# kjenike/panagram

Hardware: AMD Instinct MI355X
Metric: anchored k-mers/sec building pan-kmer bitmap (higher is better)
Workload: dtype u64

## Files before the change

### panagram_amd/csrc/pg_anchor.hip

```cpp
#include "pg_kernels.h"

#ifndef PG_ANCHOR_PART
#define PG_ANCHOR_PART -1
#endif
#define PG_HAS_PART(n) (PG_ANCHOR_PART == -1 || PG_ANCHOR_PART == (n))
#define PG_MAIN_PART (PG_ANCHOR_PART <= 0)
#if defined(PG_PHASE_TIMING) && PG_ANCHOR_PART != -1
#error "a -DPG_PHASE_TIMING build keeps its counters in one device variable: compile pg_anchor.hip as ONE unit (PG_ANCHOR_PART unset)"
#endif

namespace pg {

hipError_t probe_part0(hipStream_t s, uint32_t w, uint32_t ntiles, const SubTable &st, const uint64_t *seqw, const uint32_t *nmw, const uint32_t *has_n,
                       const SeqDesc *sd, const AnchorDesc *ad, const uint32_t *tile_contig, const uint32_t *sched, uint32_t tile_base, uint8_t *out1,
                       uint32_t nbytes, const RowCols &rc, int rowmode, const FuseArgs *fuse);
hipError_t probe_part1(hipStream_t s, uint32_t w, uint32_t ntiles, const SubTable &st, const uint64_t *seqw, const uint32_t *nmw, const uint32_t *has_n,
                       const SeqDesc *sd, const AnchorDesc *ad, const uint32_t *tile_contig, const uint32_t *sched, uint32_t tile_base, uint8_t *out1,
                       uint32_t nbytes, const RowCols &rc, int rowmode, const FuseArgs *fuse);
hipError_t probe_part2(hipStream_t s, uint32_t w, uint32_t ntiles, const SubTable &st, const uint64_t *seqw, const uint32_t *nmw, const uint32_t *has_n,
                       const SeqDesc *sd, const AnchorDesc *ad, const uint32_t *tile_contig, const uint32_t *sched, uint32_t tile_base, uint8_t *out1,
                       uint32_t nbytes, const RowCols &rc, int rowmode, const FuseArgs *fuse);
hipError_t insert_part0(hipStream_t s, uint32_t win, uint32_t ntiles, const SubTable &st, int w, uint32_t bits, uint32_t count_mode, const uint64_t *seqw,
                        const uint32_t *nmw, const uint32_t *has_n, const SeqDesc *sd, const uint32_t *tile0, uint32_t ncontigs,
                        unsigned long long *counters, uint32_t max_probe);
// ... 363 lines not shown
        for (uint32_t bb = 0; bb < rc.nb1; ++bb) row[rc.col0 + 4 + bb] = (uint8_t)(m1 >> (8 * bb));
    }
}

__device__ __forceinline__ uint32_t lane_up1(uint32_t v) {
    return (uint32_t)__builtin_amdgcn_update_dpp((int)v, (int)v, 0x138 , 0xf, 0xf, false);
}
__device__ __forceinline__ unsigned long long differs_from_lane_below(uint32_t v) {
    uint32_t t;
    asm("s_nop 1\n\tv_xor_b32_dpp %0, %1, %1 wave_shr:1 row_mask:0xf bank_mask:0xf" : "=&v"(t) : "v"(v));
    return __builtin_amdgcn_ballot_w64(t != 0u);
}
#define PG_DPPMIN "s_nop 1\n\tv_min_u32_dpp %0, %0, %1 wave_shr:1 row_mask:0xf bank_mask:0xf\n\t"
template <int W>
__device__ __forceinline__ uint32_t sliding_min(uint32_t x) {
    uint32_t m = x;
    if constexpr (W == 2) asm(PG_DPPMIN : "+v"(m) : "v"(x));
    if constexpr (W == 3) asm(PG_DPPMIN PG_DPPMIN : "+v"(m) : "v"(x));
    if constexpr (W == 4) asm(PG_DPPMIN PG_DPPMIN PG_DPPMIN : "+v"(m) : "v"(x));
    if constexpr (W == 5) asm(PG_DPPMIN PG_DPPMIN PG_DPPMIN PG_DPPMIN : "+v"(m) : "v"(x));
    if constexpr (W == 6) asm(PG_DPPMIN PG_DPPMIN PG_DPPMIN PG_DPPMIN PG_DPPMIN : "+v"(m) : "v"(x));
    if constexpr (W == 7) asm(PG_DPPMIN PG_DPPMIN PG_DPPMIN PG_DPPMIN PG_DPPMIN PG_DPPMIN : "+v"(m) : "v"(x));
    if constexpr (W == 8) asm(PG_DPPMIN PG_DPPMIN PG_DPPMIN PG_DPPMIN PG_DPPMIN PG_DPPMIN PG_DPPMIN : "+v"(m) : "v"(x));
    static_assert(W >= 1 && W <= 8, "minimizer window");
    return m;
}
#undef PG_DPPMIN
__device__ __forceinline__ uint32_t suffix_min8_row(uint32_t x) {
    uint32_t r = x;
    asm("s_nop 1\n\tv_min_u32_dpp %0, %0, %0 row_shl:1 row_mask:0xf bank_mask:0xf\n\t"
        "s_nop 1\n\tv_min_u32_dpp %0, %0, %0 row_shl:2 row_mask:0xf bank_mask:0xf\n\t"
        "s_nop 1\n\tv_min_u32_dpp %0, %0, %0 row_shl:4 row_mask:0xf bank_mask:0xf"
        : "+v"(r));
    return r;
}
#define PG_F "v_min_u32_dpp %0, %0, %0 wave_shr:1 row_mask:0xf bank_mask:0xf\n\t"
#define PG_S(n) "v_min_u32_dpp %1, %1, %1 row_shl:" #n " row_mask:0xf bank_mask:0xf\n\t"
#define PG_N0 "s_nop 0\n\t"
#define PG_N1 "s_nop 1\n\t"
template <int W>
__device__ __forceinline__ uint32_t sliding_min_suffix(uint32_t x, uint32_t &suffix) {
    uint32_t m = x, r = suffix;
    static_assert(W >= 2 && W <= 8, "minimizer window");
    if constexpr (W == 2) asm(PG_N1 PG_F PG_S(1) PG_N1 PG_S(2) PG_N1 PG_S(4) : "+v"(m), "+v"(r));
    if constexpr (W == 3) asm(PG_N1 PG_F PG_S(1) PG_N0 PG_F PG_S(2) PG_N1 PG_S(4) : "+v"(m), "+v"(r));
    if constexpr (W == 4) asm(PG_N1 PG_F PG_S(1) PG_N0 PG_F PG_S(2) PG_N0 PG_F PG_S(4) : "+v"(m), "+v"(r));
    if constexpr (W == 5) asm(PG_N1 PG_F PG_S(1) PG_N0 PG_F PG_S(2) PG_N0 PG_F PG_S(4) PG_N0 PG_F : "+v"(m), "+v"(r));
    if constexpr (W == 6) asm(PG_N1 PG_F PG_S(1) PG_N0 PG_F PG_S(2) PG_N0 PG_F PG_S(4) PG_N0 PG_F PG_N1 PG_F : "+v"(m), "+v"(r));
    if constexpr (W == 7) asm(PG_N1 PG_F PG_S(1) PG_N0 PG_F PG_S(2) PG_N0 PG_F PG_S(4) PG_N0 PG_F PG_N1 PG_F PG_N1 PG_F : "+v"(m), "+v"(r));
    if constexpr (W == 8) asm(PG_N1 PG_F PG_S(1) PG_N0 PG_F PG_S(2) PG_N0 PG_F PG_S(4) PG_N0 PG_F PG_N1 PG_F PG_N1 PG_F PG_N1 PG_F : "+v"(m), "+v"(r));
    suffix = r;
    return m;
}
#undef PG_F
#undef PG_S
#undef PG_N0
#undef PG_N1
__device__ __forceinline__ uint32_t lanes_le_index(unsigned long long mask, uint32_t base) {
    const unsigned long long m1 = mask >> 1;
    const uint32_t c = base + (uint32_t)(mask & 1ull) - 1u;
    return __builtin_amdgcn_mbcnt_hi((uint32_t)(m1 >> 32), __builtin_amdgcn_mbcnt_lo((uint32_t)m1, c));
}

__device__ __forceinline__ uint32_t run_ids(unsigned long long lmask) {
    const uint32_t below = __builtin_amdgcn_mbcnt_hi((uint32_t)(lmask >> 32), __builtin_amdgcn_mbcnt_lo((uint32_t)lmask, ~0u));
    uint32_t rid;
    unsigned long long carry_out;
    asm("v_addc_co_u32_e64 %0, %1, %2, 0, %3" : "=v"(rid), "=s"(carry_out) : "v"(below), "s"(lmask));
    return rid;
}
__device__ __forceinline__ uint32_t set_lane_index(unsigned long long mask, uint32_t base) {
    return __builtin_amdgcn_mbcnt_hi((uint32_t)(mask >> 32), __builtin_amdgcn_mbcnt_lo((uint32_t)mask, base));
}

__device__ __forceinline__ void cols_or_position(unsigned long long *cols, uint32_t pl, uint32_t m0) {
    while (m0) {
        const uint32_t j = (uint32_t)__ffs((int)m0) - 1u;
        m0 &= m0 - 1u;
        atomicOr(&cols[(pl >> 6) * COLS_G + j], 1ull << (pl & 63u));
    }
}

template <bool TWO, int ROWMODE, int SLOTS, int MAXRUN, bool WIDE, int LEVELS, bool INL = false>
__device__ __forceinline__ void drain_queue(const SubTable &st, uint32_t qn, const uint64_t *sw, const uint64_t *rw, uint32_t *q_line,
                                            uint32_t *q_step, uint16_t *q_pl, uint32_t *lines_w, uint4 *buf,
                                            uint8_t *tile_rows, uint32_t nbytes, const RowCols rc, int lane) {
    const int k = (int)st.k;
    constexpr int LDS_LINE_U4 = SLOTS + 1;
    constexpr int STAGE_ITERS = (MAXRUN * SLOTS + 63) / 64;
    const uint8_t *chunk_base = st.buckets + (uint32_t)(lane % SLOTS) * 16u;
    const uint32_t lbytes = INL ? st.layout * 64u : st.slots * (WIDE ? 8u : 16u);
    static_assert(LEVELS >= 1, "k_probe's entries (home line, group) are turned into (next line, step) by level 1's staged batches");
    for (int level = 1; qn > 0; ++level) {
        __syncthreads();
        if (level > LEVELS) {
            for (uint32_t e = lane; e < qn; e += 64) {
                uint32_t m0, m1;
                const uint64_t key = canonical_from_le(extract_bases(sw, q_pl[e]), k);
                if constexpr (WIDE && INL) {
                    uint32_t rw4[4];
                    lane_chase_inl(st, key, (uint32_t)level, q_line[e], q_step[e], rw4);
                    if (rw4[0] | rw4[1] | rw4[2] | rw4[3]) store_row_regs(tile_rows + (uint64_t)q_pl[e] * nbytes, nbytes, rw4);
                } else if constexpr (WIDE) {
                    lane_chase_wide(st, key, (uint32_t)level, q_line[e], q_step[e], m0, m1);
                    if (m1) store_row_wide(st.masks, st.W, nbytes, tile_rows + (uint64_t)q_pl[e] * nbytes, m0, m1);
                } else {
                    lane_chase<TWO, SLOTS>(st, key, (uint32_t)level, q_line[e], q_step[e], m0, m1);
                    if constexpr (ROWMODE == 3) cols_or_position(reinterpret_cast<unsigned long long *>(tile_rows), q_pl[e], m0);
                    else if (m0 | m1) store_row<ROWMODE>(tile_rows + (uint64_t)q_pl[e] * nbytes, m0, m1, rc);
                }
            }
            break;
        }
        uint32_t kept = 0;
        for (uint32_t i0 = 0; i0 < qn; i0 += 64) {
            const uint32_t e = i0 + lane;
            const bool act = e < qn;
            const uint32_t ec = act ? e : qn - 1;
            uint32_t line = q_line[ec], step = q_step[ec];
            if (GROUP_CHAIN > 1 && level == 1) {
                step = step_of_group(step, st.nbuckets);
                line = next_line(line, step, st.nbuckets);
            }
            const uint32_t pl = q_pl[ec];
            const uint64_t kmask = kmer_mask(k);
            const uint64_t X = extract_bases32(reinterpret_cast<const uint32_t *>(sw), pl) & kmask;
            const uint64_t key = canonical_from_xb(X, revcomp_window(rw, pl, kmask, PROBE_SEQ_BASES - (uint32_t)k), k);
            const uint32_t prev_line = lane_up1(line);
            const bool leader = act && (lane == 0 || line != prev_line);
            const unsigned long long lmask = __builtin_amdgcn_ballot_w64(leader);
            const uint32_t rid = lanes_le_index(lmask, 0u);
            const uint32_t nruns = (uint32_t)__popcll(lmask);
            uint32_t m0 = 0, m1 = 0;
            [[maybe_unused]] uint32_t rw4[4] = {0, 0, 0, 0};
            int rcode = 0;
            const uint32_t padline = lmask ? (uint32_t)__builtin_amdgcn_readlane((int)line, __builtin_ctzll(lmask)) : 0u;
            for (uint32_t r0 = 0; r0 < nruns; r0 += MAXRUN) {
                const uint32_t nl = min((uint32_t)MAXRUN, nruns - r0);
                if (lane < MAXRUN) lines_w[lane] = padline;
                if (leader && rid - r0 < nl) lines_w[rid - r0] = line;
                __syncthreads();
                uint4 v[STAGE_ITERS];
                uint32_t ln[STAGE_ITERS];
#pragma unroll
                for (int u = 0; u < STAGE_ITERS; ++u) ln[u] = lines_w[u * (64 / SLOTS) + lane / SLOTS];
#pragma unroll
                for (int u = 0; u < STAGE_ITERS; ++u) v[u] = *reinterpret_cast<const uint4 *>(chunk_base + (uint64_t)ln[u] * lbytes);
#pragma unroll
                for (int u = 0; u < STAGE_ITERS; ++u) {
                    const uint32_t idx = u * 64 + lane;
                    if constexpr (WIDE) buf[(idx / SLOTS) * LDS_LINE_U4 + (idx % SLOTS)] = v[u];
                    else stage_chunk(buf + (idx / SLOTS) * LDS_LINE_U4, idx % SLOTS, SLOTS, v[u]);
                }
                __syncthreads();
                if (act && rid - r0 < nl) {
                    if constexpr (WIDE && INL) {
                        rcode = scan_keys_inl(buf + (rid - r0) * LDS_LINE_U4, key, st.slots, m1);
                        if (m1) masks_inl(buf + (rid - r0) * LDS_LINE_U4, st.slots, st.W, m1 - 1u, rw4);
                    } else if constexpr (WIDE) {
                        rcode = scan_keys16_lds(buf + (rid - r0) * LDS_LINE_U4, key, m1);
                        m0 = line;
                    } else {
                        rcode = scan_line_lds<TWO, SLOTS>(buf + (rid - r0) * LDS_LINE_U4, key, m0, m1);
                    }
                }
                __syncthreads();
            }
            const bool again = act && rcode < 0;
            if constexpr (WIDE && INL) {
                if (act && m1) store_row_regs(tile_rows + (uint64_t)pl * nbytes, nbytes, rw4);
            } else if constexpr (WIDE) {
                if (act && m1) store_row_wide(st.masks, st.W, nbytes, tile_rows + (uint64_t)pl * nbytes, m0, m1);
            } else {
                if constexpr (ROWMODE == 3) {
                    if (act) cols_or_position(reinterpret_cast<unsigned long long *>(tile_rows), pl, m0);
                } else {
                    if (act && (m0 | m1)) store_row<ROWMODE>(tile_rows + (uint64_t)pl * nbytes, m0, m1, rc);
                }
            }
            const unsigned long long kmask2 = __builtin_amdgcn_ballot_w64(again);
            if (again) {
                const uint32_t slot = set_lane_index(kmask2, kept);
                uint32_t nl2 = line, ns2 = step;
                if constexpr (LEVELS + 1 < (int)GROUP_CHAIN) nl2 = next_line(line, step, st.nbuckets);
                else advance_line(key, (uint32_t)level + 1, st.nbuckets, nl2, ns2);
                q_line[slot] = nl2;
                q_step[slot] = ns2;
                q_pl[slot] = (uint16_t)pl;
            }
            kept += (uint32_t)__popcll(kmask2);
            __syncthreads();
        }
        qn = kept;
    }
}

#ifndef PG_FUSE_LOAD_SC1
#define PG_FUSE_LOAD_SC1 1
#endif
typedef const __attribute__((address_space(1))) uint8_t *GlobalBytes;
template <int NW>
__device__ __forceinline__ void fuse_load_row(GlobalBytes base, uint32_t off, uint32_t (&w)[NW]) {
    GlobalBytes p = base + off;
#if PG_FUSE_LOAD_SC1
#pragma unroll
    for (int i = 0; i + 1 < NW; i += 2) {
        const unsigned long long v = __hip_atomic_load(reinterpret_cast<const __attribute__((address_space(1))) unsigned long long *>(p + 4 * i), __ATOMIC_RELAXED,
                                                       __HIP_MEMORY_SCOPE_AGENT);
        w[i] = (uint32_t)v, w[i + 1] = (uint32_t)(v >> 32);
    }
    if constexpr (NW & 1)
        w[NW - 1] = __hip_atomic_load(reinterpret_cast<const __attribute__((address_space(1))) uint32_t *>(p + 4 * (NW - 1)), __ATOMIC_RELAXED, __HIP_MEMORY_SCOPE_AGENT);
#else
    const WordsN<NW> v = *reinterpret_cast<const __attribute__((address_space(1))) WordsN<NW> *>(p);
#pragma unroll
    for (int i = 0; i < NW; ++i) w[i] = v.w[i];
#endif
}
__device__ __forceinline__ void fuse_flush_word(const uint32_t (&pl)[5], uint32_t *out16, int lane) {
    uint32_t R[16];
#pragma unroll
    for (int q = 0; q < 8; ++q) {
        uint32_t v = 0;
#pragma unroll
        for (int i = 0; i < 5; ++i) v |= ((pl[i] >> q) & 0x01010101u) << i;
        R[2 * q] = v & 0x00FF00FFu;
        R[2 * q + 1] = (v >> 8) & 0x00FF00FFu;
    }
#define PG_XCHG(HALF, BIT)                                                  \
    {                                                                       \
        const bool up = (lane & BIT) != 0;                                  \
        _Pragma("unroll") for (int i = 0; i < HALF; ++i) {                  \
            const uint32_t send = up ? R[i] : R[i + HALF];                  \
            const uint32_t keep = up ? R[i + HALF] : R[i];                  \
            R[i] = keep + (uint32_t)__shfl_xor((int)send, BIT);             \
        }                                                                   \
    }
    PG_XCHG(8, 32)
    PG_XCHG(4, 16)
    PG_XCHG(2, 8)
    PG_XCHG(1, 4)
#undef PG_XCHG
    R[0] += (uint32_t)__shfl_xor((int)R[0], 2);
    R[0] += (uint32_t)__shfl_xor((int)R[0], 1);
    if ((lane & 3) == 0) {
        const uint32_t idx = (uint32_t)lane >> 2;
        out16[(idx >> 1) + ((idx & 1u) ? 8u : 0u)] = R[0];
    }
}
template <int NWP, bool LASTPASS>
__device__ __forceinline__ void tile_statistics_pass(uint32_t *Hc, GlobalBytes rs, uint32_t npos, uint32_t nbytes, uint32_t woff,
                                                     uint32_t keep_last, uint32_t split, uint32_t N, uint32_t (&pcs)[4], uint32_t *cs_out, int lane) {
    const uint32_t N1 = N + 1u;
    uint32_t ones[NWP], twos[NWP], fours[NWP], eights[NWP], sixteens[NWP], hold4[NWP], hold8[NWP];
#pragma unroll
    for (int w = 0; w < NWP; ++w) ones[w] = twos[w] = fours[w] = eights[w] = sixteens[w] = hold4[w] = hold8[w] = 0;
    uint32_t nx[4][NWP];
    auto request = [&](int g, uint32_t (&dst)[4][NWP]) __attribute__((always_inline)) {
#pragma unroll
        for (int i = 0; i < 4; ++i) {
            const uint32_t r = (uint32_t)(4 * g + i) * 64u + (uint32_t)lane;
            fuse_load_row<NWP>(rs, min(r, npos - 1u) * nbytes + woff, dst[i]);
        }
    };
    request(0, nx);
#pragma unroll
    for (int g = 0; g < 4; ++g) {
        uint32_t rw[4][NWP];
#pragma unroll
        for (int i = 0; i < 4; ++i)
// ... 53 lines not shown
        const uint32_t pl[5] = {ones[w], twos[w], fours[w], eights[w], sixteens[w]};
        fuse_flush_word(pl, cs_out + 16 * w, lane);
    }
}

template <int NW>
__device__ __forceinline__ void tile_statistics(uint32_t *H, const uint8_t *tile_rows, uint32_t npos, uint32_t nbytes, const AnchorDesc &a,
                                                uint32_t tile_start, uint32_t tile, const FuseArgs &fo, int lane) {
    const uint32_t N = fo.ngenomes, N1 = N + 1u, hw = fo.hw;
    const uint32_t nh = 2u * N1;
#ifdef PG_PHASE_TIMING
    uint32_t tph[5] = {0, 0, 0, 0, 0}, tph_t = (uint32_t)__builtin_readcyclecounter();
#define PG_TPH(i) { const uint32_t n_ = (uint32_t)__builtin_readcyclecounter(); tph[i] += n_ - tph_t; tph_t = n_; }
#else
#define PG_TPH(i)
#endif
    __builtin_amdgcn_s_waitcnt(0x0F70);
    __syncthreads();
    PG_TPH(0)
    const uint64_t base = reinterpret_cast<uint64_t>(tile_rows);
    GlobalBytes rs = reinterpret_cast<GlobalBytes>(((uint64_t)(uint32_t)__builtin_amdgcn_readfirstlane((int)(uint32_t)(base >> 32)) << 32) |
                                                   (uint32_t)__builtin_amdgcn_readfirstlane((int)(uint32_t)base));
    const uint32_t r100 = (100u - tile_start % 100u) % 100u + 100u * (uint32_t)lane;
    const bool want100 = fo.out100 != nullptr && r100 < npos;
    uint32_t w100[NW];
    fuse_load_row<NW>(rs, min(r100, npos - 1u) * nbytes, w100);
    for (uint32_t i = lane; i < 4u * nh; i += 64) H[i] = 0;
    const uint64_t bin_end = ((uint64_t)(tile_start / a.binlen) + 1u) * a.binlen;
    const uint32_t split = (uint32_t)min((uint64_t)npos, bin_end - tile_start);
    const uint32_t keep = (nbytes & 3u) ? ((1u << (8u * (nbytes & 3u))) - 1u) : ~0u;
    uint32_t *const Hc = H + ((uint32_t)lane & 3u) * nh;
    uint32_t *cs_out = fo.tile_cs + (uint64_t)tile * fo.csw;
    uint32_t pcs[4] = {0, 0, 0, 0};
    __syncthreads();
    PG_TPH(1)
    if constexpr (NW <= 2) {
        tile_statistics_pass<NW, true>(Hc, rs, npos, nbytes, 0u, keep, split, N, pcs, cs_out, lane);
        PG_TPH(2)
    } else {
        tile_statistics_pass<2, false>(Hc, rs, npos, nbytes, 0u, ~0u, split, N, pcs, cs_out, lane);
        PG_TPH(2)
        tile_statistics_pass<NW - 2, true>(Hc, rs, npos, nbytes, 8u, keep, split, N, pcs, cs_out + 32, lane);
    }
    if (want100) {
        uint8_t *dst = fo.out100 + a.out100_off + (uint64_t)((tile_start + r100) / 100u) * nbytes;
#pragma unroll
        for (int i = 0; i < NW; ++i)
#pragma unroll
            for (int b = 0; b < 4; ++b)
                if ((uint32_t)(4 * i + b) < nbytes) dst[4 * i + b] = (uint8_t)(w100[i] >> (8 * b));
    }
    __syncthreads();
    PG_TPH(3)
    uint32_t *th = fo.tile_hist + (uint64_t)tile * hw;
    for (uint32_t i = lane; i < hw; i += 64) {
        const uint32_t lo = H[2u * i] + H[nh + 2u * i] + H[2u * nh + 2u * i] + H[3u * nh + 2u * i];
        const uint32_t hi = H[2u * i + 1u] + H[nh + 2u * i + 1u] + H[2u * nh + 2u * i + 1u] + H[3u * nh + 2u * i + 1u];
        th[i] = lo | (hi << 16);
    }
    PG_TPH(4)
#ifdef PG_PHASE_TIMING
    if (lane == 0)
        for (int i = 0; i < 5; ++i) atomicAdd(&pg_phase_cycles[(blockIdx.x & 1023u) * 16u + 11 + i], (unsigned long long)tph[i]);
#endif
#undef PG_TPH
}

template <bool TWO, int ROWMODE, int SLOTS, bool WIDE>
constexpr bool probe_pipelined = SLOTS == 8 && !WIDE && ROWMODE != 3 && (ROWMODE == 1 || ROWMODE >= 4 || TWO);
template <int W_C, bool TWO, int ROWMODE, int SLOTS, bool M64, bool WIDE = false, bool INL = false, bool FUSE = false>
__global__ __launch_bounds__(64, ((probe_pipelined<TWO, ROWMODE, SLOTS, WIDE> || INL || FUSE) ? 8 : 1))
__attribute__((amdgpu_num_sgpr(80))) void k_probe(const SubTable st, const uint64_t *__restrict__ seqw,
                                              const uint32_t *__restrict__ nmw, const uint32_t *__restrict__ has_n,
                                              const SeqDesc *__restrict__ sd, const AnchorDesc *__restrict__ ad,
                                              const uint32_t *__restrict__ tile_contig,
                                              const uint32_t *__restrict__ sched, uint32_t tile_base,
                                              uint8_t *__restrict__ out1, uint32_t nbytes, const RowCols rc, const FuseArgs fo) {
    constexpr int LDS_LINE_U4 = SLOTS + 1;
    constexpr int MAXRUN = PROBE_MAXRUN;
    constexpr int STAGE_ITERS = (MAXRUN * SLOTS + 63) / 64;
    constexpr int BUF_U4 = ((STAGE_ITERS * 64 + SLOTS - 1) / SLOTS) * LDS_LINE_U4;
    constexpr int OFF_RW = PROBE_SEQW * 8, OFF_NW = OFF_RW + (PROBE_SEQW + 1) * 8, OFF_LW = OFF_NW + PROBE_SEQW * 4;
    constexpr int QCAP = PROBE_QCAP;
    constexpr int OFF_BUF = (OFF_LW + MAXRUN * 4 + 15) & ~15, OFF_QL = OFF_BUF + BUF_U4 * 16, OFF_QS = OFF_QL + QCAP * 4;
    constexpr int OFF_QP = OFF_QS + QCAP * 4, LDS_BYTES = OFF_QP + QCAP * 2;
    static_assert(OFF_LW <= 1020 || PROBE_TILE > 1024, "the sequence words must stay within reach of ds_read2_b32's offsets");
    __shared__ __attribute__((aligned(16))) uint8_t lds[LDS_BYTES];
    uint64_t *const sw = reinterpret_cast<uint64_t *>(lds);
    uint64_t *const rw = reinterpret_cast<uint64_t *>(lds + OFF_RW);
    uint32_t *const nw = reinterpret_cast<uint32_t *>(lds + OFF_NW);
    uint32_t(*const lines_w)[MAXRUN] = reinterpret_cast<uint32_t(*)[MAXRUN]>(lds + OFF_LW);
    uint4(*const buf)[BUF_U4] = reinterpret_cast<uint4(*)[BUF_U4]>(lds + OFF_BUF);
    uint32_t *const q_line = reinterpret_cast<uint32_t *>(lds + OFF_QL);
    uint32_t *const q_step = reinterpret_cast<uint32_t *>(lds + OFF_QS);
    uint16_t *const q_pl = reinterpret_cast<uint16_t *>(lds + OFF_QP);
    PG_PH_DECL
    const int lane = threadIdx.x;
    const int k = (int)st.k;
    if constexpr (W_C != 0) __builtin_assume(k >= 20 && k <= 32);
    const uint32_t tile = sched ? sched[blockIdx.x + tile_base] : blockIdx.x + tile_base;
    const uint32_t c = tile_contig[tile];
    const AnchorDesc a = ad[c];
    const SeqDesc s = sd[c];
    const uint32_t tile_start = (tile - a.tile0) * PROBE_TILE;
    const uint32_t npos = min((uint32_t)PROBE_TILE, a.nkmers - tile_start);
    const bool hasn = has_n[c] != 0;

    for (int i = lane; i < PROBE_SEQW; i += 64) {
        const uint64_t wi = (uint64_t)(tile_start >> 5) + i;
        const uint64_t wv = wi < s.nwords ? seqw[s.seq_off + wi] : 0ull;
        sw[i] = wv;
        rw[PROBE_SEQW - 1 - i] = pair_reverse64(~wv);
        nw[i] = (hasn && wi < s.nwords) ? nmw[s.seq_off + wi] : 0u;
    }
    if (lane == 0) rw[PROBE_SEQW] = 0;
    __syncthreads();

    const uint64_t kmask = W_C ? (((uint64_t)(k == 32 ? ~0u : ((1u << (2 * k - 32)) - 1u)) << 32) | 0xFFFFFFFFull) : kmer_mask(k);
    const uint32_t rcb = PROBE_SEQ_BASES - (uint32_t)k;
    constexpr int HALO = W_C ? W_C - 1 : 0;
    constexpr bool CARRY = W_C >= 2;
    constexpr bool CUT = W_C != 0;
    const uint32_t m = W_C ? (uint32_t)k - W_C + 1 : 0;
    const uint64_t mm64 = (m >= 32) ? ~0ull : ((1ull << (2 * (m ? m : 1))) - 1);
    __shared__ unsigned long long cols[ROWMODE == 3 ? TILE_SLOTS * COLS_G : 1];
    if constexpr (ROWMODE == 3) {
        for (uint32_t i = lane; i < TILE_SLOTS * COLS_G; i += 64) cols[i] = 0;
        __syncthreads();
    }
#if PG_ABLATE == 9 || PG_ABLATE == 10
    uint8_t *tile_rows = out1 + (uint64_t)(blockIdx.x & 255u) * PROBE_TILE * nbytes;
#else
    uint8_t *tile_rows = ROWMODE == 3 ? reinterpret_cast<uint8_t *>(cols) : out1 + a.out_off + (uint64_t)tile_start * nbytes;
#endif
    uint32_t qn = 0;

    const uint8_t *chunk_base = st.buckets + (uint32_t)(lane % SLOTS) * 16u;
    const uint32_t lbytes = INL ? st.layout * 64u : st.slots * (WIDE ? 8u : 16u);

    struct Front {
        uint64_t key;
        uint32_t grp, line, rid, nruns, padline;
        uint32_t adv;
        uint32_t ln[STAGE_ITERS];
        unsigned long long rmask, amask, lmask;
    };
    auto carry_at = [&](const uint32_t b0) __attribute__((always_inline)) {
        uint32_t y = ~0u;
        if constexpr (CARRY) {
            const uint32_t q = b0 + (uint32_t)min(lane, HALO - 1);
            const uint64_t fa = extract_bases32(reinterpret_cast<const uint32_t *>(sw), q) & mm64;
            const uint64_t fr = extract_bases32(reinterpret_cast<const uint32_t *>(rw), PROBE_SEQ_BASES - q - m) & mm64;
            const uint32_t h = M64 ? mmer_rank(fa < fr ? fa : fr) : mz_order(min((uint32_t)fa, (uint32_t)fr));
            y = h;
        }
        return y;
    };
    uint32_t carry = ~0u;
    auto front = [&](const uint32_t b0) __attribute__((always_inline)) {
        Front f;
        const int32_t pl = (int32_t)(b0 + lane);
        f.rmask = __builtin_amdgcn_ballot_w64(pl < (int32_t)npos);
        const uint32_t pq = (uint32_t)pl;
        const uint64_t X = extract_bases32(reinterpret_cast<const uint32_t *>(sw), pq) & kmask;
        const uint64_t B = revcomp_window(rw, pq, kmask, rcb);
        f.key = ~(X > B ? X : B) & kmask;
        f.amask = f.rmask;
        if (hasn) f.amask &= __builtin_amdgcn_ballot_w64(extract_nmask(nw, pq, k) == 0);
        [[maybe_unused]] uint32_t own = 0;
        if (W_C) {
            constexpr uint32_t off = (uint32_t)HALO;
            if constexpr (!M64) {
                const uint32_t mm32 = (uint32_t)mm64;
                const uint32_t fa = __builtin_amdgcn_alignbit((uint32_t)(X >> 32), (uint32_t)X, 2 * off) & mm32;
                const uint32_t fr = __builtin_amdgcn_alignbit((uint32_t)(B >> 32), (uint32_t)B, 2 * (HALO - off)) & mm32;
                f.grp = mz_order(min(fa, fr));
            } else {
// ... 51 lines not shown
        return f;
    };
    struct Lines {
        uint4 v[STAGE_ITERS];
    };
    auto issue = [&](const Front &f, const uint32_t r0) __attribute__((always_inline)) {
        Lines L;
        uint32_t ln[STAGE_ITERS];
        if (r0 != 0u) {
            const uint32_t nl = min((uint32_t)MAXRUN, f.nruns - r0);
            const bool leader = __builtin_amdgcn_inverse_ballot_w64(f.lmask);
            if (lane < MAXRUN) lines_w[0][lane] = f.padline;
            if (leader && f.rid - r0 < nl) lines_w[0][f.rid - r0] = f.line;
            __syncthreads();
        }
#pragma unroll
        for (int it = 0; it < STAGE_ITERS; ++it) {
            if (r0 != 0u) ln[it] = lines_w[0][it * (64 / SLOTS) + lane / SLOTS];
            else ln[it] = f.ln[it];
#if PG_ABLATE == 1
            ln[it] &= 511u;
#endif
        }
#pragma unroll
        for (int it = 0; it < STAGE_ITERS; ++it) L.v[it] = *reinterpret_cast<const uint4 *>(chunk_base + (uint64_t)ln[it] * lbytes);
        return L;
    };
    auto back = [&](const Front &f, const Lines &L, const uint32_t b0, auto &&after_staging) __attribute__((always_inline)) {
        const bool act = __builtin_amdgcn_inverse_ballot_w64(f.amask), inrange = __builtin_amdgcn_inverse_ballot_w64(f.rmask);
        const int32_t pl = (int32_t)(b0 + lane);
        uint32_t m0 = 0, m1 = 0;
        [[maybe_unused]] uint32_t rw4[4] = {0, 0, 0, 0};
        int rcode = 0;
        auto stage = [&](const Lines &S) __attribute__((always_inline)) {
            uint4 *const mine = buf[0] + ((uint32_t)lane / SLOTS) * LDS_LINE_U4;
#pragma unroll
            for (int it = 0; it < STAGE_ITERS; ++it) {
                if constexpr (WIDE) mine[it * (64 / SLOTS) * LDS_LINE_U4 + ((uint32_t)lane % SLOTS)] = S.v[it];
                else stage_chunk(mine + it * (64 / SLOTS) * LDS_LINE_U4, (uint32_t)lane % SLOTS, SLOTS, S.v[it]);
            }
            __syncthreads();
        };
        auto scan = [&](const uint32_t r0) __attribute__((always_inline)) {
            const uint32_t nl = min((uint32_t)MAXRUN, f.nruns - r0);
#if PG_ABLATE == 5
            if (act && f.rid - r0 < nl) {
                rcode = 1;
                m0 = m1 = reinterpret_cast<const uint32_t *>(buf[0] + (f.rid - r0) * LDS_LINE_U4)[2];
            }
#else
            if (act && f.rid - r0 < nl) {
                if constexpr (WIDE && INL) {
                    rcode = scan_keys_inl(buf[0] + (f.rid - r0) * LDS_LINE_U4, f.key, st.slots, m1);
                    if (m1) masks_inl(buf[0] + (f.rid - r0) * LDS_LINE_U4, st.slots, st.W, m1 - 1u, rw4);
                } else if constexpr (WIDE) {
                    rcode = scan_keys16_lds(buf[0] + (f.rid - r0) * LDS_LINE_U4, f.key, m1);
                    m0 = f.line;
                } else {
                    rcode = scan_line_lds<TWO, SLOTS>(buf[0] + (f.rid - r0) * LDS_LINE_U4, f.key, m0, m1);
                }
            }
#endif
            __syncthreads();
        };
        PG_PH(1)
        __builtin_amdgcn_s_waitcnt(0x0F70);
        PG_PH(2)
        stage(L);
        PG_PH(3)
        after_staging();
        PG_PH(4)
        scan(0u);
        PG_PH(5)
        if constexpr (!CUT)
        for (uint32_t r0 = MAXRUN; r0 < f.nruns; r0 += MAXRUN) {
            const Lines X = issue(f, r0);
            __builtin_amdgcn_s_waitcnt(0x0F70);
            stage(X);
            scan(r0);
        }
        const unsigned long long omask = f.amask & __builtin_amdgcn_sicmp(rcode, 0, 40);
        const bool ovf = __builtin_amdgcn_inverse_ballot_w64(omask);
        if (omask) {
            uint32_t step, nx;
            if constexpr (GROUP_CHAIN == 1) {
                key_sequence(f.key, st.nbuckets, nx, step);
            } else {
                step = f.grp;
                nx = f.line;
            }
            const uint32_t slot = set_lane_index(omask, qn);
            if (ovf) {
                q_line[slot] = nx;
                q_step[slot] = step;
                q_pl[slot] = (uint16_t)pl;
            }
            qn += (uint32_t)__popcll(omask);
        }
        PG_PH(10)
        if constexpr (WIDE && INL) {
            const bool fuse = (nbytes & 3u) != 0u && b0 + (uint32_t)__popcll(f.rmask) < npos;
            if (fuse) {
                const uint32_t mine = inrange ? rw4[0] : 0u;
                const uint32_t nxt = (uint32_t)__builtin_amdgcn_update_dpp(0, (int)mine, 0x130 , 0xf, 0xf, true);
                if (inrange) store_row_fused(tile_rows + (uint64_t)(uint32_t)pl * nbytes, nbytes, rw4, nxt);
            } else if (inrange) {
                store_row_regs(tile_rows + (uint64_t)(uint32_t)pl * nbytes, nbytes, rw4);
            }
        } else if constexpr (WIDE) {
#if PG_ABLATE == 2
            if (inrange && m0 == 0xDEADBEEFu && m1 == 77u)
#elif PG_ABLATE == 8 || PG_ABLATE == 10
            if (m1) m0 = 0, m1 = 1;
            if (inrange)
#else
            if (st.W == 4u && (nbytes & 3u) != 0u && b0 + (uint32_t)__popcll(f.rmask) < npos) {
                uint32_t v4[4] = {0, 0, 0, 0};
                if (inrange && m1) {
                    const WordsN<4> g = *reinterpret_cast<const WordsN<4> *>(reinterpret_cast<const uint32_t *>(st.masks) + ((uint64_t)m0 * SPLIT_KEYS + (m1 - 1u)) * 4u);
                    v4[0] = g.w[0], v4[1] = g.w[1], v4[2] = g.w[2], v4[3] = g.w[3];
                }
                const uint32_t nxt = (uint32_t)__builtin_amdgcn_update_dpp(0, (int)v4[0], 0x130 , 0xf, 0xf, true);
                if (inrange) store_row_fused(tile_rows + (uint64_t)(uint32_t)pl * nbytes, nbytes, v4, nxt);
            } else if (inrange)
#endif
                store_row_wide(st.masks, st.W, nbytes, tile_rows + (uint64_t)(uint32_t)pl * nbytes, m0, m1);
        } else if constexpr (ROWMODE == 3) {
            const uint32_t w0 = b0 >> 6, sh = b0 & 63u;
            for (uint32_t j = 0; j < rc.col0; ++j) {
                const unsigned long long shifted = __ballot(inrange && ((m0 >> j) & 1u));
                if (lane == 0 && shifted) {
                    cols[w0 * COLS_G + j] |= shifted << sh;
                    if (sh && (shifted >> (64u - sh))) cols[(w0 + 1) * COLS_G + j] |= shifted >> (64u - sh);
                }
            }
        } else {
            if (ROWMODE == 6 && b0 + (uint32_t)__popcll(f.rmask) < npos) {
                const uint32_t mine = inrange ? m0 : 0u;
                const uint32_t nxt = (uint32_t)__builtin_amdgcn_update_dpp(0, (int)mine, 0x130 , 0xf, 0xf, true);
                struct __attribute__((packed)) U32 { uint32_t v; };
                if (inrange) reinterpret_cast<U32 *>(tile_rows + (uint32_t)pl * 3u)->v = (m0 & 0xFFFFFFu) | (nxt << 24);
            } else if constexpr (ROWMODE == 6) {
                const uint32_t nxt = (uint32_t)__builtin_amdgcn_update_dpp(0, (int)m0, 0x130 , 0xf, 0xf, false);
                const uint32_t o4 = (uint32_t)reinterpret_cast<uintptr_t>(tile_rows) & 3u;
                const uint32_t j = ((uint32_t)pl - o4) & 3u;
                const uint32_t lo = (nxt << 24) | (m0 & 0xFFFFFFu);
                const uint32_t dw = __builtin_amdgcn_alignbit(nxt >> 8, lo, 8u * j);
                const unsigned long long nextin = f.rmask >> 1;
                const unsigned long long dmask = f.rmask & nextin & __builtin_amdgcn_ballot_w64(j != 3u);
                const unsigned long long fmask = f.rmask & (1ull | ~nextin);
                uint8_t *row = tile_rows + (uint32_t)pl * 3u;
                if (__builtin_amdgcn_inverse_ballot_w64(dmask)) *reinterpret_cast<uint32_t *>(row + j) = dw;
                if (__builtin_amdgcn_inverse_ballot_w64(fmask)) store_row<ROWMODE>(row, m0, m1, rc);
            } else
#if PG_ABLATE == 2
            if (inrange && m0 == 0xDEADBEEFu)
#else
            if (ROWMODE == 0 && TWO && rc.words == 3u && nbytes >= 5u && b0 + (uint32_t)__popcll(f.rmask) < npos) {
                const uint32_t mine = inrange ? m0 : 0u;
                const uint32_t nxt = (uint32_t)__builtin_amdgcn_update_dpp(0, (int)mine, 0x130 , 0xf, 0xf, true);
                if (inrange) {
                    typedef uint32_t u32x2u __attribute__((ext_vector_type(2), aligned(1)));
                    const uint32_t t8 = 8u * (nbytes - 4u);
                    u32x2u q = {m0, (m1 & ((1u << t8) - 1u)) | (nxt << t8)};
                    *reinterpret_cast<u32x2u *>(tile_rows + (uint32_t)pl * nbytes) = q;
                }
            } else if (inrange)
#endif
                store_row<ROWMODE>(tile_rows + (ROWMODE == 1 ? (uint32_t)pl : ROWMODE == 4 ? (uint32_t)pl * 4u : ROWMODE == 5 ? (uint32_t)pl * 2u : ROWMODE == 6 ? (uint32_t)pl * 3u : (uint32_t)pl * nbytes), m0, m1, rc);
        }
        PG_PH(6)
    };
    constexpr bool PIPE = probe_pipelined<TWO, ROWMODE, SLOTS, WIDE>;
    constexpr int LEVELS = (W_C >= 6 && !TWO && !WIDE && PROBE_STAGED_LEVELS > 1) ? 1 : PROBE_STAGED_LEVELS;
    static_assert(QCAP >= 128, "an early drain must leave room for a batch");
    constexpr uint32_t QROOM = QCAP - 64;
    uint32_t b0 = 0;
    if constexpr (PIPE) {
        Lines L;
#pragma unroll
        for (int it = 0; it < STAGE_ITERS; ++it) L.v[it] = make_uint4(0, 0, 0, 0);
        PG_PH(0)
        carry = carry_at(0u);
        Front cur = front(0u);
        L = issue(cur, 0u);
        for (;;) {
            PG_PH(7)
            const uint32_t b1 = b0 + cur.adv;
            const bool more = b1 < npos;
            Front nxt = cur;
            __builtin_amdgcn_sched_barrier(0);
            if (more) nxt = front(b1);
            __builtin_amdgcn_sched_barrier(0);
            back(cur, L, b0, [&]() __attribute__((always_inline)) {
                if (more) L = issue(nxt, 0u);
            });
            __builtin_amdgcn_sched_barrier(0);
            b0 = b1;
            if (!more || qn > QROOM) break;
            cur = nxt;
        }
    } else {
        {
            carry = carry_at(0u);
            const Front f = front(0u);
            const Lines L = issue(f, 0u);
            back(f, L, 0u, [] {});
            b0 = f.adv;
        }
        while (b0 < npos && qn <= QROOM) {
            const Front f = front(b0);
            const Lines L = issue(f, 0u);
            back(f, L, b0, [] {});
            b0 += f.adv;
        }
    }
    PG_PH(7)
    for (;;) {
        drain_queue<TWO, ROWMODE, SLOTS, MAXRUN, WIDE, LEVELS, INL>(st, qn, sw, rw, q_line, q_step, q_pl, lines_w[0], buf[0], tile_rows, nbytes, rc, lane);
        qn = 0;
        if (b0 >= npos) break;
        __syncthreads();
        carry = carry_at(b0);
        while (b0 < npos && qn <= QROOM) {
            const Front f = front(b0);
            const Lines L = issue(f, 0u);
            back(f, L, b0, [] {});
            b0 += f.adv;
        }
    }
    PG_PH(8)
    PG_PH_FLUSH
    if constexpr (FUSE) {
        static_assert(ROWMODE != 1 && ROWMODE != 3 && LDS_BYTES >= 4 * 4 * 2 * 129, "fused statistics: rows of 2..16 bytes; four copies of 2 x 129 histogram counters in LDS");
        const AnchorDesc *ad2 = ad;
        const uint32_t *tc2 = tile_contig, *sched2 = sched;
        asm volatile("" : "+s"(ad2), "+s"(tc2), "+s"(sched2));
        const uint32_t tile2 = sched2 ? sched2[blockIdx.x + tile_base] : blockIdx.x + tile_base;
        const AnchorDesc a2 = ad2[tc2[tile2]];
        if (a2.binlen >= (uint32_t)PROBE_TILE) {
            const uint32_t ts2 = (tile2 - a2.tile0) * PROBE_TILE;
            const uint32_t np2 = min((uint32_t)PROBE_TILE, a2.nkmers - ts2);
            const uint8_t *rows2 = out1 + a2.out_off + (uint64_t)ts2 * nbytes;
            uint32_t *H = reinterpret_cast<uint32_t *>(lds);
            if constexpr (WIDE) {
                if (nbytes <= 12u) tile_statistics<3>(H, rows2, np2, nbytes, a2, ts2, tile2, fo, lane);
                else tile_statistics<4>(H, rows2, np2, nbytes, a2, ts2, tile2, fo, lane);
            } else {
                tile_statistics<TWO ? 2 : 1>(H, rows2, np2, nbytes, a2, ts2, tile2, fo, lane);
            }
        }
    }
    if constexpr (ROWMODE == 3) {
        __syncthreads();
        const uint32_t width = nbytes, trel = tile - tile_base;
        unsigned long long *dst = reinterpret_cast<unsigned long long *>(out1) + (uint64_t)trel * TILE_SLOTS * width;
        for (uint32_t i = lane; i < TILE_SLOTS * width; i += 64) dst[i] = cols[(i / width) * COLS_G + i % width];
    }
}

constexpr int INSERT_QCAP = 256;

template <bool COUNT, bool CLAIM = true>
__device__ __forceinline__ int wave_insert_batch(const SubTable &st, bool valid, uint64_t key, uint32_t grp, int w, uint32_t bits,
                                                 uint32_t max_probe, int lane) {
    const uint32_t kstride = key_stride(st), slots = st.slots;
    uint32_t b = home_of_group(grp, st.nbuckets), step = step_of_group(grp, st.nbuckets), probes = 0;
    int s = -1;
    bool done = !valid, fresh = false;
    int r = 0;
    auto shfl64 = [](uint64_t v, int src) __attribute__((always_inline)) {
        return (uint64_t)(uint32_t)__shfl((int)(uint32_t)v, src) | ((uint64_t)(uint32_t)__shfl((int)(uint32_t)(v >> 32), src) << 32);
    };
    auto resolve = [&](uint32_t sl, bool claimed) __attribute__((always_inline)) {
        uint32_t *mp = mask_ptr(st, b, sl, (uint32_t)w);
        if (COUNT) {
            if (*mp < 0xFFFFFF00u) atomicAdd(mp, bits);
        } else if (claimed) {
            *reinterpret_cast<volatile uint32_t *>(mp) = bits;
        } else {
            const uint32_t cur = *mp;
            if ((cur & bits) != bits) *reinterpret_cast<volatile uint32_t *>(mp) = cur | bits;
        }
        r = claimed ? 1 : 0;
        done = true;
    };
    while (__ballot(!done)) {
        if (!done && s >= (int)slots) {
            if (++probes >= max_probe) {
                done = true;
                r = -1;
            } else {
                advance_line(key, probes, st.nbuckets, b, step);
                s = -1;
            }
        }
        if (!done && s < 0) {
            uint8_t *base = st.buckets + (uint64_t)b * line_bytes(st);
            int hit = -1, fr = -1;
            for (uint32_t s0 = 0; s0 < slots; s0 += 8) {
                uint64_t kk[8];
#pragma unroll
// ... 536 lines not shown
```

### panagram_amd/csrc/pg_device.h

```cpp
#pragma once
#include <hip/hip_runtime.h>
#include <stdint.h>
#include <math.h>

namespace pg {

constexpr uint64_t EMPTY_KEY = ~0ull;
constexpr uint64_t TOMB_KEY = ~0ull - 1;
constexpr int MAX_SUB = 1;
constexpr uint32_t MAX_WORDS = 64;

struct SubTable {
    uint8_t *buckets;
    uint64_t nbuckets;
    uint32_t W;
    uint32_t word0;
    uint32_t k;
    uint32_t m;
    uint32_t slots;
    uint32_t layout;
    uint8_t *masks;
};
constexpr uint32_t LAYOUT_SLOTS = 0, LAYOUT_SPLIT = 1, LAYOUT_INLINE = 2;
constexpr uint32_t SPLIT_KEYS = 16;
// ... 34 lines not shown
    if (load > 0.0 && load < 0.375) {
        sparse = (load / 0.375) * (load / 0.375);
        if (sparse < 0.25) sparse = 0.25;
    }
    double leff = 1.5e8;
    if (first_len) {
        leff = (double)first_len;
        double v = (double)expected_keys / (2.3 * leff);
        if (v > 1.0) leff *= sqrt(v < 16.0 ? v : 16.0);
    } else if (expected_keys) {
        leff = (double)expected_keys / 2.3;
    }
    uint32_t m_lo = 15;
    if (k - (wmax - 1) > m_lo) m_lo = k - (wmax - 1);
    if (expected_keys) {
        uint32_t mk = 15;
        while (mk < 27 && (1ull << (2 * mk)) < 4 * expected_keys) ++mk;
        if (mk - 2 > m_lo) m_lo = mk - 2;
    }
    const uint32_t m_hi = k - (MZ_WMIN - 1);
    if (m_lo > m_hi) m_lo = m_hi;
    const double wcost_co[9] = {0, 0, 0, 35.0, 19.5, 10.5, 3.5, 0.5, 0.0};
    const double wcost_one[9] = {0, 0, 0, 62.0, 42.0, 26.0, 12.0, 2.0, 0.0};
    const double *wcost = cosched == 1 ? wcost_one : wcost_co;
    uint32_t best = m_lo;
    double best_cost = 1e30;
    for (uint32_t m = m_lo; m <= m_hi; ++m) {
        const double r = (m >= 31 ? 4.6e18 : (double)(1ull << (2 * m))) / leff;
        const double relief = r >= 10.0 ? sparse : r <= 5.0 ? 1.0 : 1.0 + (sparse - 1.0) * (r - 5.0) / 5.0;
        const double c = wcost[k - m + 1] + merged * relief / r;
        if (c < best_cost) {
            best_cost = c;
            best = m;
        }
    }
    return best;
}

__host__ __device__ __forceinline__ uint32_t fmix32(uint32_t h) {
    h ^= h >> 16;
    h *= 0x85ebca6bu;
    h ^= h >> 13;
    h *= 0xc2b2ae35u;
    h ^= h >> 16;
    return h;
}
__host__ __device__ __forceinline__ uint32_t mz_order(uint32_t c) { return c * 0x9E3779B1u; }

__device__ __forceinline__ uint32_t range32(uint32_t h, uint64_t n) { return __umulhi(h, (uint32_t)n); }

__device__ __forceinline__ uint32_t group_of_key(uint64_t key) {
    return (uint32_t)key ^ fmix32((uint32_t)(key >> 32) + 0x9E3779B9u);
}
__device__ __forceinline__ uint32_t mix1(uint32_t g, uint32_t mul) {
    const uint32_t h = g * mul;
    return h ^ (h >> 15);
}
__device__ __forceinline__ uint32_t home_of_group(uint32_t g, uint64_t nlines) { return range32(g * 0x85ebca6bu, nlines); }
__device__ __forceinline__ uint32_t step_of_group(uint32_t g, uint64_t nlines) {
    return 1u + range32(mix1(g ^ 0x5bd1e995u, 0xc2b2ae35u), nlines - 1);
}
__device__ __forceinline__ uint32_t next_line(uint32_t line, uint32_t step, uint64_t nlines) {
    const uint32_t n = line + step;
    return min(n, n - (uint32_t)nlines);
}
#ifndef PG_GROUP_CHAIN
#define PG_GROUP_CHAIN 4
#endif
constexpr uint32_t GROUP_CHAIN = PG_GROUP_CHAIN;
static_assert(GROUP_CHAIN >= 1, "a group owns at least its home line");
__device__ __forceinline__ void key_sequence(uint64_t key, uint64_t nlines, uint32_t &home, uint32_t &step) {
    const uint32_t g2 = fmix32(group_of_key(key) ^ 0x7feb352du);
    home = home_of_group(g2, nlines);
    step = step_of_group(g2, nlines);
}
__device__ __forceinline__ void advance_line(uint64_t key, uint32_t level, uint64_t nlines, uint32_t &line,
                                             uint32_t &step) {
    if (level == GROUP_CHAIN) {
        key_sequence(key, nlines, line, step);
    } else {
        line = next_line(line, step, nlines);
    }
}

__device__ __forceinline__ uint64_t pair_reverse64(uint64_t x) {
    const uint32_t lo = __brev((uint32_t)(x >> 32)), hi = __brev((uint32_t)x);
    const uint32_t lo2 = ((lo >> 1) & 0x55555555u) | ((lo << 1) & ~0x55555555u);
    const uint32_t hi2 = ((hi >> 1) & 0x55555555u) | ((hi << 1) & ~0x55555555u);
    return (uint64_t)lo2 | ((uint64_t)hi2 << 32);
}
__device__ __forceinline__ uint64_t kmer_mask(int k) { return (k == 32) ? ~0ull : ((1ull << (2 * k)) - 1); }

__device__ __forceinline__ uint64_t revcomp_le(uint64_t X, int k) {
    return (pair_reverse64(~X) >> (64 - 2 * k)) & kmer_mask(k);
}
__device__ __forceinline__ uint64_t canonical_from_xb(uint64_t X, uint64_t B, int k) {
    return ~(X > B ? X : B) & kmer_mask(k);
}
__device__ __forceinline__ uint64_t canonical_from_le(uint64_t x, int k) {
    x &= kmer_mask(k);
    return canonical_from_xb(x, revcomp_le(x, k), k);
}

constexpr uint32_t SKETCH_BITS = 16;
__host__ __device__ __forceinline__ uint64_t sketch_hash(uint64_t x) {
    x ^= x >> 30;
    x *= 0xbf58476d1ce4e5b9ull;
    x ^= x >> 27;
    x *= 0x94d049bb133111ebull;
    x ^= x >> 31;
    return x;
}

__host__ __device__ __forceinline__ uint32_t mmer_rank(uint64_t c) {
    const uint32_t hi = (uint32_t)(c >> 32);
    return mz_order((uint32_t)c ^ ((hi << 11) | (hi >> 21)) ^ ((hi << 23) | (hi >> 9)));
}

__device__ __forceinline__ uint32_t minimizer_from_xb(uint64_t X, uint64_t B, uint32_t m, uint32_t w) {
    const uint64_t mm = (m >= 32) ? ~0ull : ((1ull << (2 * m)) - 1);
    uint32_t best = ~0u;
    for (uint32_t i = 0; i < w; ++i) {
        const uint64_t a = (X >> (2 * i)) & mm;
        const uint64_t b = (B >> (2 * (w - 1 - i))) & mm;
        const uint32_t h = mmer_rank(a < b ? a : b);
        best = h < best ? h : best;
    }
    return best;
}

__device__ __forceinline__ uint32_t group_of(const SubTable &st, uint64_t key) {
    if (st.m == 0) return group_of_key(key);
    const int k = (int)st.k;
    const uint64_t X = pair_reverse64(key) >> (64 - 2 * k);
    const uint64_t B = ~key & kmer_mask(k);
    return minimizer_from_xb(X, B, st.m, st.k - st.m + 1);
}

template <typename P>
__device__ __forceinline__ uint64_t extract_bases(P words, uint64_t p) {
    uint64_t w = p >> 5;
    uint32_t sh = (uint32_t)(p & 31) * 2;
    uint64_t lo = words[w];
    uint64_t hi = words[w + 1];
    return (lo >> sh) | ((hi << 1) << (63 - sh));
}

__device__ __forceinline__ uint64_t extract_bases32(const uint32_t *words32, uint32_t p) {
    const uint32_t d = p >> 4, sh = (p & 15u) * 2u;
    const uint32_t d0 = words32[d], d1 = words32[d + 1], d2 = words32[d + 2];
    const uint32_t lo = __builtin_amdgcn_alignbit(d1, d0, sh);
    const uint32_t hi = __builtin_amdgcn_alignbit(d2, d1, sh);
    return (uint64_t)lo | ((uint64_t)hi << 32);
}

template <typename P>
__device__ __forceinline__ uint32_t extract_nmask(P words, uint64_t p, int k) {
    uint64_t w = p >> 5;
    uint32_t sh = (uint32_t)(p & 31);
    uint64_t v = (uint64_t)words[w] | ((uint64_t)words[w + 1] << 32);
    v >>= sh;
    uint32_t km = (k == 32) ? 0xFFFFFFFFu : ((1u << k) - 1);
    return (uint32_t)v & km;
}
template <typename P>
__device__ __forceinline__ uint64_t extract_nmask64(P words, uint64_t p) {
// ... 88 lines not shown
```

### panagram_amd/csrc/pg_kernels.h

```cpp
#pragma once
#include "pg_device.h"

namespace pg {

#ifndef PG_PROBE_TILE
#define PG_PROBE_TILE 1024
#endif
#ifndef PG_PROBE_MAXRUN
#define PG_PROBE_MAXRUN 16
#endif
constexpr int PROBE_TILE = PG_PROBE_TILE;
constexpr int PROBE_MAXRUN = PG_PROBE_MAXRUN;
constexpr int COLS_G = 8;
constexpr uint32_t TILE_SLOTS = PROBE_TILE / 64;
static_assert(PROBE_TILE % 512 == 0, "the column kernels take a tile in units of 512 positions");
#ifndef PG_PROBE_STAGED_LEVELS
#define PG_PROBE_STAGED_LEVELS 2
#endif
constexpr int PROBE_STAGED_LEVELS = PG_PROBE_STAGED_LEVELS;
#ifndef PG_PROBE_QCAP
#define PG_PROBE_QCAP 192
#endif
constexpr int PROBE_QCAP = PG_PROBE_QCAP;

struct RowCols {
    uint32_t col0, nb0, nb1, words;
};

struct SeqDesc {
    uint64_t seq_off;
    uint64_t nwords;
    uint64_t len;
};

struct AnchorDesc {
    uint64_t out_off;
    uint64_t out100_off;
    uint64_t bin_off;
    uint32_t nkmers;
    uint32_t binlen;
    uint32_t tile0;
    uint32_t nbins;
};

hipError_t launch_table_init(hipStream_t st, const SubTable &t);
struct TextChunk {
    uint64_t off;
    uint32_t len, rec;
};
hipError_t launch_text_pack(hipStream_t st, const uint8_t *d_text, const TextChunk *d_chunks, uint64_t nchunks,
                            const uint64_t *d_rec_chunk0, uint32_t nrec, uint32_t *d_counts, uint64_t *d_base,
                            uint64_t *d_rec_len, const SeqDesc *sd, uint64_t *seqw, uint32_t *nmw, uint32_t *has_n);
hipError_t launch_text_headers(hipStream_t st, const uint8_t *d_text, uint64_t nbytes, uint64_t *d_out, uint32_t cap, uint32_t *d_count);
hipError_t launch_seq_tailmask(hipStream_t st, const SeqDesc *sd, uint32_t n, uint64_t *seqw, uint32_t *nmw);
struct SeqCopy {
    const uint64_t *src_seqw;
    const uint32_t *src_nmw;
    const uint32_t *src_has_n;
    uint64_t src_off, dst_off, nwords;
};
hipError_t launch_seq_gather(hipStream_t st, const SeqCopy *jobs, uint32_t n, uint64_t max_words, uint64_t *seqw, uint32_t *nmw,
                             uint32_t *has_n);
hipError_t launch_pack(hipStream_t st, const void *d_ascii, uint64_t len, uint64_t *seqw, uint32_t *nmw,
                       uint64_t nwords, uint32_t *has_n);
hipError_t launch_sketch(hipStream_t st, int k, const uint64_t *seqw, const uint32_t *nmw, const uint32_t *has_n,
                         uint64_t nkmers, uint32_t *regs);
constexpr uint32_t SKETCH_JOB = 1u << 16;
hipError_t launch_sketch_set(hipStream_t st, int k, const SeqDesc *sd, const uint2 *jobs, uint32_t njobs, const uint64_t *seqw,
                             const uint32_t *nmw, const uint32_t *has_n, uint32_t *regs);
constexpr int MINHASH_K = 21;
constexpr uint32_t MINHASH_JOB = 1u << 16;
hipError_t launch_minhash(hipStream_t st, const SeqDesc *sd, const uint2 *jobs, uint32_t njobs, const uint64_t *seqw,
                          const uint32_t *nmw, const uint32_t *has_n, uint64_t limit, uint32_t seed, uint64_t *cand, uint64_t cap,
                          unsigned long long *count, unsigned long long *bases);
hipError_t launch_insert_seq(hipStream_t st, const SubTable &t, int w, uint32_t bits, int k,
                             const uint64_t *seqw, const uint32_t *nmw, const uint32_t *has_n,
                             uint64_t nkmers, unsigned long long *counters, uint32_t max_probe, int count_mode = 0);
hipError_t launch_insert_tiles(hipStream_t st, const SubTable &t, int w, uint32_t bits, int count_mode, const uint64_t *seqw,
                               const uint32_t *nmw, const uint32_t *has_n, const SeqDesc *sd, const uint32_t *tile0,
                               uint32_t ncontigs, uint32_t ntiles, unsigned long long *counters, uint32_t max_probe);
hipError_t preload_table_kernels();
hipError_t preload_anchor_kernels();
hipError_t preload_rows_kernels();
hipError_t preload_deflate_kernels();
hipError_t launch_tile0(hipStream_t st, const SeqDesc *sd, uint32_t n, uint32_t k, uint32_t tile, uint32_t *tile0);
hipError_t launch_count_spill(hipStream_t st, const SubTable &t, unsigned long long *counters);
hipError_t launch_merge_min(hipStream_t st, const SubTable &src, const SubTable &dst, int w, uint32_t bits,
                            uint32_t min_count, unsigned long long *counters, uint32_t max_probe);
hipError_t launch_insert_keys(hipStream_t st, const SubTable &t, int w, const uint64_t *keys,
                              const uint32_t *vals, uint64_t n, unsigned long long *counters,
                              uint32_t max_probe);
hipError_t launch_import_kmc(hipStream_t st, const SubTable &t, int w, const uint8_t *rec, uint64_t first_record, uint64_t nrec,
                             const uint64_t *lut, uint64_t nlut, uint32_t prefixes_per_bin, uint32_t suffix_bytes,
                             uint32_t counter_bytes, uint32_t min_count, uint32_t max_count, unsigned long long *counters,
                             uint32_t max_probe, uint32_t phase = 2, uint32_t dense_above = 0);
hipError_t launch_rehash(hipStream_t st, const SubTable &src, const SubTable &dst,
                         unsigned long long *counters, uint32_t max_probe, uint32_t ngenomes);
hipError_t launch_export(hipStream_t st, const SubTable &t, int w, uint64_t *keys, uint32_t *vals,
                         uint64_t cap, unsigned long long *count);
hipError_t launch_counters(hipStream_t st, const SubTable &t, int w, int k, const uint64_t *seqw,
                           const uint32_t *nmw, const uint32_t *has_n, uint64_t nkmers, uint32_t *out);
struct FuseArgs {
    uint8_t *out100;
    uint32_t *tile_hist;
// ... 83 lines not shown
```

Measured before the change: 234.0 billion.

## Store only group id in probe overflow queue and recompute line per level

The overflow queue in LDS now keeps only the group id and position for each k-mer instead of a line and a step. At every drain level the probe line and step are recomputed from the group, or from the key once past the group chain. This cuts per-entry LDS from ten to six bytes, and the queue capacity is raised to use the freed space so fewer drain rounds are needed. In exchange it adds arithmetic to recompute lines at each level.

```diff
diff --git a/panagram_amd/csrc/pg_anchor.hip b/panagram_amd/csrc/pg_anchor.hip
--- a/panagram_amd/csrc/pg_anchor.hip
+++ b/panagram_amd/csrc/pg_anchor.hip
@@ -469,30 +469,32 @@
 }
 
 template <bool TWO, int ROWMODE, int SLOTS, int MAXRUN, bool WIDE, int LEVELS, bool INL = false>
-__device__ __forceinline__ void drain_queue(const SubTable &st, uint32_t qn, const uint64_t *sw, const uint64_t *rw, uint32_t *q_line,
-                                            uint32_t *q_step, uint16_t *q_pl, uint32_t *lines_w, uint4 *buf,
+__device__ __forceinline__ void drain_queue(const SubTable &st, uint32_t qn, const uint64_t *sw, const uint64_t *rw, uint32_t *q_grp,
+                                            uint16_t *q_pl, uint32_t *lines_w, uint4 *buf,
                                             uint8_t *tile_rows, uint32_t nbytes, const RowCols rc, int lane) {
     const int k = (int)st.k;
     constexpr int LDS_LINE_U4 = SLOTS + 1;
     constexpr int STAGE_ITERS = (MAXRUN * SLOTS + 63) / 64;
     const uint8_t *chunk_base = st.buckets + (uint32_t)(lane % SLOTS) * 16u;
     const uint32_t lbytes = INL ? st.layout * 64u : st.slots * (WIDE ? 8u : 16u);
-    static_assert(LEVELS >= 1, "k_probe's entries (home line, group) are turned into (next line, step) by level 1's staged batches");
+    static_assert(LEVELS >= 1, "k_probe's entries (group, position) get their line and step from level 1's staged batches");
     for (int level = 1; qn > 0; ++level) {
         __syncthreads();
         if (level > LEVELS) {
             for (uint32_t e = lane; e < qn; e += 64) {
                 uint32_t m0, m1;
                 const uint64_t key = canonical_from_le(extract_bases(sw, q_pl[e]), k);
+                uint32_t cl, cs;
+                line_of_level(q_grp[e], key, (uint32_t)level, st.nbuckets, cl, cs);
                 if constexpr (WIDE && INL) {
                     uint32_t rw4[4];
-                    lane_chase_inl(st, key, (uint32_t)level, q_line[e], q_step[e], rw4);
+                    lane_chase_inl(st, key, (uint32_t)level, cl, cs, rw4);
                     if (rw4[0] | rw4[1] | rw4[2] | rw4[3]) store_row_regs(tile_rows + (uint64_t)q_pl[e] * nbytes, nbytes, rw4);
                 } else if constexpr (WIDE) {
-                    lane_chase_wide(st, key, (uint32_t)level, q_line[e], q_step[e], m0, m1);
+                    lane_chase_wide(st, key, (uint32_t)level, cl, cs, m0, m1);
                     if (m1) store_row_wide(st.masks, st.W, nbytes, tile_rows + (uint64_t)q_pl[e] * nbytes, m0, m1);
                 } else {
-                    lane_chase<TWO, SLOTS>(st, key, (uint32_t)level, q_line[e], q_step[e], m0, m1);
+                    lane_chase<TWO, SLOTS>(st, key, (uint32_t)level, cl, cs, m0, m1);
                     if constexpr (ROWMODE == 3) cols_or_position(reinterpret_cast<unsigned long long *>(tile_rows), q_pl[e], m0);
                     else if (m0 | m1) store_row<ROWMODE>(tile_rows + (uint64_t)q_pl[e] * nbytes, m0, m1, rc);
                 }
@@ -504,15 +506,19 @@
             const uint32_t e = i0 + lane;
             const bool act = e < qn;
             const uint32_t ec = act ? e : qn - 1;
-            uint32_t line = q_line[ec], step = q_step[ec];
-            if (GROUP_CHAIN > 1 && level == 1) {
-                step = step_of_group(step, st.nbuckets);
-                line = next_line(line, step, st.nbuckets);
-            }
+            const uint32_t grp = q_grp[ec];
             const uint32_t pl = q_pl[ec];
             const uint64_t kmask = kmer_mask(k);
             const uint64_t X = extract_bases32(reinterpret_cast<const uint32_t *>(sw), pl) & kmask;
             const uint64_t key = canonical_from_xb(X, revcomp_window(rw, pl, kmask, PROBE_SEQ_BASES - (uint32_t)k), k);
+            uint32_t line, step;
+            if constexpr (LEVELS < (int)GROUP_CHAIN) {
+                line = home_of_group(grp, st.nbuckets);
+                step = step_of_group(grp, st.nbuckets);
+                for (int i = 0; i < level; ++i) line = next_line(line, step, st.nbuckets);
+            } else {
+                line_of_level(grp, key, (uint32_t)level, st.nbuckets, line, step);
+            }
             const uint32_t prev_line = lane_up1(line);
             const bool leader = act && (lane == 0 || line != prev_line);
             const unsigned long long lmask = __builtin_amdgcn_ballot_w64(leader);
@@ -568,11 +574,7 @@
             const unsigned long long kmask2 = __builtin_amdgcn_ballot_w64(again);
             if (again) {
                 const uint32_t slot = set_lane_index(kmask2, kept);
-                uint32_t nl2 = line, ns2 = step;
-                if constexpr (LEVELS + 1 < (int)GROUP_CHAIN) nl2 = next_line(line, step, st.nbuckets);
-                else advance_line(key, (uint32_t)level + 1, st.nbuckets, nl2, ns2);
-                q_line[slot] = nl2;
-                q_step[slot] = ns2;
+                q_grp[slot] = grp;
                 q_pl[slot] = (uint16_t)pl;
             }
             kept += (uint32_t)__popcll(kmask2);
@@ -792,8 +794,8 @@
     constexpr int BUF_U4 = ((STAGE_ITERS * 64 + SLOTS - 1) / SLOTS) * LDS_LINE_U4;
     constexpr int OFF_RW = PROBE_SEQW * 8, OFF_NW = OFF_RW + (PROBE_SEQW + 1) * 8, OFF_LW = OFF_NW + PROBE_SEQW * 4;
     constexpr int QCAP = PROBE_QCAP;
-    constexpr int OFF_BUF = (OFF_LW + MAXRUN * 4 + 15) & ~15, OFF_QL = OFF_BUF + BUF_U4 * 16, OFF_QS = OFF_QL + QCAP * 4;
-    constexpr int OFF_QP = OFF_QS + QCAP * 4, LDS_BYTES = OFF_QP + QCAP * 2;
+    constexpr int OFF_BUF = (OFF_LW + MAXRUN * 4 + 15) & ~15, OFF_QG = OFF_BUF + BUF_U4 * 16;
+    constexpr int OFF_QP = OFF_QG + QCAP * 4, LDS_BYTES = OFF_QP + QCAP * 2;
     static_assert(OFF_LW <= 1020 || PROBE_TILE > 1024, "the sequence words must stay within reach of ds_read2_b32's offsets");
     __shared__ __attribute__((aligned(16))) uint8_t lds[LDS_BYTES];
     uint64_t *const sw = reinterpret_cast<uint64_t *>(lds);
@@ -801,8 +803,7 @@
     uint32_t *const nw = reinterpret_cast<uint32_t *>(lds + OFF_NW);
     uint32_t(*const lines_w)[MAXRUN] = reinterpret_cast<uint32_t(*)[MAXRUN]>(lds + OFF_LW);
     uint4(*const buf)[BUF_U4] = reinterpret_cast<uint4(*)[BUF_U4]>(lds + OFF_BUF);
-    uint32_t *const q_line = reinterpret_cast<uint32_t *>(lds + OFF_QL);
-    uint32_t *const q_step = reinterpret_cast<uint32_t *>(lds + OFF_QS);
+    uint32_t *const q_grp = reinterpret_cast<uint32_t *>(lds + OFF_QG);
     uint16_t *const q_pl = reinterpret_cast<uint16_t *>(lds + OFF_QP);
     PG_PH_DECL
     const int lane = threadIdx.x;
@@ -1020,17 +1021,9 @@
         const unsigned long long omask = f.amask & __builtin_amdgcn_sicmp(rcode, 0, 40);
         const bool ovf = __builtin_amdgcn_inverse_ballot_w64(omask);
         if (omask) {
-            uint32_t step, nx;
-            if constexpr (GROUP_CHAIN == 1) {
-                key_sequence(f.key, st.nbuckets, nx, step);
-            } else {
-                step = f.grp;
-                nx = f.line;
-            }
             const uint32_t slot = set_lane_index(omask, qn);
             if (ovf) {
-                q_line[slot] = nx;
-                q_step[slot] = step;
+                q_grp[slot] = f.grp;
                 q_pl[slot] = (uint16_t)pl;
             }
             qn += (uint32_t)__popcll(omask);
@@ -1155,7 +1148,7 @@
     }
     PG_PH(7)
     for (;;) {
-        drain_queue<TWO, ROWMODE, SLOTS, MAXRUN, WIDE, LEVELS, INL>(st, qn, sw, rw, q_line, q_step, q_pl, lines_w[0], buf[0], tile_rows, nbytes, rc, lane);
+        drain_queue<TWO, ROWMODE, SLOTS, MAXRUN, WIDE, LEVELS, INL>(st, qn, sw, rw, q_grp, q_pl, lines_w[0], buf[0], tile_rows, nbytes, rc, lane);
         qn = 0;
         if (b0 >= npos) break;
         __syncthreads();
diff --git a/panagram_amd/csrc/pg_device.h b/panagram_amd/csrc/pg_device.h
--- a/panagram_amd/csrc/pg_device.h
+++ b/panagram_amd/csrc/pg_device.h
@@ -140,6 +140,17 @@
         line = next_line(line, step, nlines);
     }
 }
+__device__ __forceinline__ void line_of_level(uint32_t grp, uint64_t key, uint32_t level, uint64_t nlines, uint32_t &line,
+                                              uint32_t &step) {
+    uint32_t g = grp, n = level;
+    if (level >= GROUP_CHAIN) {
+        g = fmix32(group_of_key(key) ^ 0x7feb352du);
+        n = level - GROUP_CHAIN;
+    }
+    line = home_of_group(g, nlines);
+    step = step_of_group(g, nlines);
+    for (uint32_t i = 0; i < n; ++i) line = next_line(line, step, nlines);
+}
 
 __device__ __forceinline__ uint64_t pair_reverse64(uint64_t x) {
     const uint32_t lo = __brev((uint32_t)(x >> 32)), hi = __brev((uint32_t)x);
diff --git a/panagram_amd/csrc/pg_kernels.h b/panagram_amd/csrc/pg_kernels.h
--- a/panagram_amd/csrc/pg_kernels.h
+++ b/panagram_amd/csrc/pg_kernels.h
@@ -19,7 +19,7 @@
 #endif
 constexpr int PROBE_STAGED_LEVELS = PG_PROBE_STAGED_LEVELS;
 #ifndef PG_PROBE_QCAP
-#define PG_PROBE_QCAP 192
+#define PG_PROBE_QCAP 320
 #endif
 constexpr int PROBE_QCAP = PG_PROBE_QCAP;
 
```

After: 236.7 billion, median of 6. 1.01x the previous value.
